# DTolm/VkFFT

Measured on NVIDIA H100. Metric: batched 1D C2C FP32 throughput (sample_0 sweep N=2^7..2^22, fwd+inv), higher is better.
Workload: dtype f32

## Files before the change

vkfft_b200/csrc/kernel_inst.cuh:

```cuda
#pragma once
#include <cstdio>

#include "kernel_registry.h"
#include "stockham.cuh"
#include "generic.cuh"
#include "pipe.cuh"
#include "fused4.cuh"
#include "ew.cuh"

#if !defined(B2_EMU)
#include <cuda_runtime.h>
#endif

namespace b200fft {

#if !defined(B2_EMU)
inline int launch_checked(const void* kernel, unsigned grid, unsigned threads, size_t smem, void* stream, const b2_pass_params* P) {
    void* args[] = {const_cast<b2_pass_params*>(P)};
    return (int)cudaLaunchKernel(kernel, dim3(grid), dim3(threads), args, smem, (cudaStream_t)stream);
}
#endif

template <int KIND> struct KindTraits;
template <> struct KindTraits<B2_KIND_ROWS> {
    static constexpr int LMAP = MAP_TFAST, SMAP = MAP_TFAST, LAYOUT = LAY_LINE;
    static constexpr bool IN_UNIT = true, OUT_UNIT = true;
};
template <> struct KindTraits<B2_KIND_ROWS_TOUT> {
    static constexpr int LMAP = MAP_TFAST, SMAP = MAP_QFAST, LAYOUT = LAY_LINE;
    static constexpr bool IN_UNIT = true, OUT_UNIT = false;
// ... 404 lines not shown
        for (int s = 0; s < SchB::ns; ++s) info.radices_b[s] = SchB::r(s);
        info.launch = &fused_launch_impl<CA, CB>;
        info.prepare = &fused_prepare_impl<CA, CB>;
        info.name = name;
        b2_register_fused(&info);
    }
};
template <bool EN, typename T, int TPLA, int QA, class SchA, int TPLB, int QB, class SchB, int REGS>
struct MaybeFused {
    explicit MaybeFused(const char*) {}
};
template <typename T, int TPLA, int QA, class SchA, int TPLB, int QB, class SchB, int REGS>
struct MaybeFused<true, T, TPLA, QA, SchA, TPLB, QB, SchB, REGS> {
    FusedRegistrar<T, false, TPLA, QA, SchA, TPLB, QB, SchB, REGS> f;
    FusedRegistrar<T, true, TPLA, QA, SchA, TPLB, QB, SchB, REGS> i;
    explicit MaybeFused(const char* n) : f(n), i(n) {}
};
}
#define B2_R(...) ::b200fft::RList<__VA_ARGS__>
#define B2_KF(shard, T, REGS, TPLA, QA, SA, TPLB, QB, SB)                                                  \
    static ::b200fft::MaybeFused<B2_SHARD_ON(shard), T, TPLA, QA, SA, TPLB, QB, SB, REGS>                  \
        B2_CAT(b2_regf_, __COUNTER__)("FUSED4<" #T ";A " #TPLA "x" #QA " " #SA ";B " #TPLB "x" #QB " " #SB ">");

namespace b200fft {
template <typename T, int Q, int REGS, bool INV, int N>
struct StagedRegistrar {
    using KT = KindTraits<B2_KIND_ROWS>;
    using C = KCfg<T, RList<N>, 1, Q, 1, KT::LMAP, KT::SMAP, KT::LAYOUT, INV, 0, KT::IN_UNIT, KT::OUT_UNIT, REGS, 10>;
    b2_kernel_info info;
    explicit StagedRegistrar(const char* name) {
        info = b2_kernel_info{};
        info.kind = B2_KIND_ROWS; info.prec = PrecOf<T>::value; info.n = N; info.inv = INV; info.ops = 0;
        info.threads = C::THREADS; info.q = Q; info.tpl = 1; info.v = 1; info.smem_bytes = C::SMEM_BYTES;
        info.ns = 1; info.radices[0] = N; info.lut_size = 0;
        info.launch = &launch_impl<C>;
        info.prepare = &prepare_impl<C>;
        info.name = name;
        b2_register_kernel(&info);
    }
};
template <bool EN, typename T, int Q, int REGS, int N>
struct MaybeStaged {
    explicit MaybeStaged(const char*) {}
};
template <typename T, int Q, int REGS, int N>
struct MaybeStaged<true, T, Q, REGS, N> {
// ... 25 lines not shown
```

vkfft_b200/csrc/kernel_registry.cpp:

```cpp
#include "kernel_registry.h"

#include <cstdio>
#include <cstdlib>
#include <cstring>
#include <vector>

namespace {
std::vector<b2_kernel_info*>& table() {
    static std::vector<b2_kernel_info*> t;
    return t;
}
int variant_override(int kind, int prec, int n) {
    const char* e = getenv("B200FFT_VARIANTS");
    if (!e) return 0;
    for (const char* p = e; *p;) {
        int k, pr, nn, v, used = 0;
        if (sscanf(p, "%d:%d:%d=%d%n", &k, &pr, &nn, &v, &used) == 4) {
            if (k == kind && pr == prec && nn == n) return v;
            p += used;
        } else {
            break;
        }
        if (*p == ',') ++p;
    }
// ... 42 lines not shown
}
extern "C" const b2_fused_info* b2_find_fused_variant(int prec, int n1, int n2, int inv, int variant) {
    for (const b2_fused_info* k : ftable())
        if (k->prec == prec && k->n1 == n1 && k->n2 == n2 && k->inv == inv && k->variant == variant) return k;
    return nullptr;
}
extern "C" const b2_fused_info* b2_find_fused(int prec, int n1, int n2, int inv) {
    int v = 0;
    if (const char* e = getenv("B200FFT_FUSED_VARIANTS")) {
        for (const char* p = e; *p;) {
            int a, b, vv, used = 0;
            if (sscanf(p, "%dx%d=%d%n", &a, &b, &vv, &used) == 3) {
                if (a == n1 && b == n2) v = vv;
                p += used;
            } else break;
            if (*p == ',') ++p;
        }
    }
    const b2_fused_info* k = v ? b2_find_fused_variant(prec, n1, n2, inv, v) : nullptr;
    return k ? k : b2_find_fused_variant(prec, n1, n2, inv, 0);
}
extern "C" int b2_fused_count(void) { return (int)ftable().size(); }
extern "C" const b2_fused_info* b2_fused_at(int i) { return ftable()[i]; }
```

vkfft_b200/csrc/kernel_registry.h:

```cpp
#pragma once
#include "pass_params.h"

#ifdef __cplusplus
extern "C" {
#endif

enum {
    B2_KIND_ROWS = 0,
    B2_KIND_ROWS_TOUT = 1,
    B2_KIND_COLS = 2,
    B2_KIND_GENERIC = 3,
    B2_KIND_ELEMENTWISE = 4,
    B2_KIND_COUNT
};
enum { B2_PREC_F32 = 0, B2_PREC_F64 = 1 };

typedef struct b2_kernel_info {
    int kind, prec, n, inv, ops;
    int variant;
    int pipelined;
    int threads, q, tpl, v, smem_bytes;
    int ns;
    int radices[8];
    int lut_size;
// ... 16 lines not shown
void b2_register_kernel(const b2_kernel_info* k);
const b2_kernel_info* b2_find_kernel(int kind, int prec, int n, int inv, int ops);
const b2_kernel_info* b2_find_kernel_variant(int kind, int prec, int n, int inv, int ops, int variant);
int b2_kernel_count(void);
const b2_kernel_info* b2_kernel_at(int i);

typedef struct b2_fused_info {
    int prec, n1, n2, inv;
    int variant;
    int threads, qa, qb, smem_bytes;
    int regs;
    int ns_a, ns_b;
    int radices_a[8], radices_b[8];
    int (*launch)(const b2_fused_params* F, unsigned max_ctas, void* stream);
    int (*prepare)(void);
    const char* name;
} b2_fused_info;
void b2_register_fused(const b2_fused_info* k);
const b2_fused_info* b2_find_fused(int prec, int n1, int n2, int inv);
const b2_fused_info* b2_find_fused_variant(int prec, int n1, int n2, int inv, int variant);
int b2_fused_count(void);
const b2_fused_info* b2_fused_at(int i);

#ifdef __cplusplus
}
#endif
```

vkfft_b200/csrc/kernels_shard.cu:

```cuda
#include "kernel_inst.cuh"

#ifndef B2_SHARD
#error "compile with -DB2_SHARD=<k>"
#endif

#include "kernel_list.def"
#include "kernel_list_nonpow2.def"
#include "kernel_list_blue1.def"
#include "kernel_list_fused.def"
```

vkfft_b200/csrc/pass_params.h:

```cpp
#pragma once
#include <stdint.h>

#ifdef __cplusplus
extern "C" {
#endif

enum {
    B2_MAX_OUTER = 3,
};

enum {
    B2_OP_NONE = 0,
    B2_OP_TWIDDLE_OUT = 1,
    B2_OP_SCALE = 2,
    B2_OP_MUL_IN = 4,
    B2_OP_MUL_OUT = 8,
    B2_OP_REAL_EVEN = 16,
    B2_OP_DCT23 = 32,
    B2_OP_PERM_IN = 64,
    B2_OP_BLUESTEIN = 256,
    B2_OP_CONV = 512,
    B2_OP_BLUE_FUSED = 1024,
    B2_OP_HALF_IN = 2048,
    B2_OP_HALF_OUT = 4096,
// ... 58 lines not shown
    uint32_t gen_flags;
} b2_pass_params;

enum {
    B2_GEN_FUSE_IN = 1,
    B2_GEN_FUSE_OUT = 2,
};

typedef struct b2_fused_params {
    unsigned long long tmap_a[16]
#if defined(__GNUC__) || defined(__CUDACC__)
        __attribute__((aligned(64)))
#endif
        ;
    b2_pass_params A, B;
    uint32_t* ctl;
    uint32_t nseq;
    uint32_t U, NU;
    uint32_t R;
    uint32_t TA, TB;
    uint32_t reserved;
} b2_fused_params;

enum {
    B2_FCTL_MAX_GROUPS = 1024,
    B2_FCTL_WORDS = 64 * B2_FCTL_MAX_GROUPS,
};

#ifdef __cplusplus
}
#endif
```

vkfft_b200/csrc/plan.h:

```cpp
#pragma once
#include <stdint.h>

#include <string>
#include <vector>

#include "../../include/b200fft.h"
#include "kernel_registry.h"
#include "pass_params.h"

namespace b200fft {

enum {
    R_SUCCESS = 0,
    R_MALLOC_FAILED = 1,
    R_PLAN_NOT_INITIALIZED = 4,
    R_NULL_TEMP_PASSED = 5,
    R_FFTDIM_GT_MAX = 7,
    R_INVALID_DEVICE = 1002,
    R_ONLY_FORWARD = 1006,
    R_ONLY_INVERSE = 1007,
    R_EMPTY_FFTDIM = 2001,
    R_EMPTY_SIZE = 2002,
    R_EMPTY_BUFFER = 2004,
    R_EMPTY_TEMPBUFFER = 2006,
// ... 27 lines not shown

struct AuxSpec {
    int prec, kind;
    uint64_t a, b;
};

struct PassPlan {
    const b2_kernel_info* k = nullptr;
    const b2_kernel_info* k_unaligned = nullptr;
    b2_pass_params P{};
    unsigned grid = 0;
    int in_role = ROLE_BUFFER, out_role = ROLE_BUFFER;
    int64_t in_off = 0, out_off = 0;
    int lut_id = -1;
    int lut_id_unaligned = -1;
    int tw_id = -1;
    int aux0_id = -1, aux1_id = -1;
    int aux0_role = -1;
    bool sync_before = false;
    bool in_scalar = false, out_scalar = false;
    const b2_fused_info* fused = nullptr;
    uint32_t fz_nseq = 0, fz_U = 0, fz_NU = 0, fz_R = 0, fz_TA = 0, fz_TB = 0, fz_L = 1;
    int lut_id_plain = -1;
    std::string note;
};

struct PlanGraph {
    b200fft_desc desc{};
    int prec = 0;
    uint64_t stride[B200FFT_MAX_DIMS] = {0, 0, 0, 0};
    uint64_t batches = 1;
    uint64_t batch_stride = 0;
    uint64_t total_elems = 0;
    uint64_t temp_elems = 0;
    bool has_fwd = false, has_inv = false;
    std::vector<PassPlan> fwd, inv;
    std::vector<LutSpec> luts;
    std::vector<TwSpec> tws;
    std::vector<AuxSpec> auxs;
    uint64_t temp_elems_real = 0;
    double flops = 0;
    uint64_t algorithmic_bytes = 0;
    uint32_t axis_uploads[2][B200FFT_MAX_DIMS] = {{0, 0, 0, 0}, {0, 0, 0, 0}};
    int skip_axis = -1;
    uint64_t ctl_words = 0;
    bool role_half[ROLE_COUNT] = {false, false, false, false, false};
// ... 7 lines not shown
```

vkfft_b200/csrc/planner.cpp:

```cpp
#include <algorithm>
#include <cmath>
#include <cstdio>
#include <cstdlib>
#include <cstring>

#include "lut.h"
#include "plan.h"

namespace b200fft {
namespace {

struct Dim {
    uint64_t n;
    int64_t is, os;
};

int lut_for(PlanGraph& g, const std::vector<int>& r) {
    for (size_t i = 0; i < g.luts.size(); ++i)
        if (g.luts[i].prec == g.prec && g.luts[i].radices == r) return (int)i;
    g.luts.push_back(LutSpec{g.prec, r});
    return (int)g.luts.size() - 1;
}
int tw_for(PlanGraph& g, uint64_t M) {
    for (size_t i = 0; i < g.tws.size(); ++i)
// ... 588 lines not shown
    if (a.P.nb[1] != 1 || a.P.nb[2] != 1 || (a.P.nb[0] > 1 && a.P.in_bs[0] != (int64_t)((uint64_t)a.P.n * b.P.n)) || a.P.in_gs != 1) return;
    const uint64_t N = (uint64_t)a.P.n * b.P.n, esz = esize(g), seq_bytes = N * esz;
    const uint64_t ga = (a.P.G + fk->qa - 1) / fk->qa, gb = (b.P.G + fk->qb - 1) / fk->qb;
    uint64_t K = std::max<uint64_t>(std::max(ga, gb) / 2, 8);
    if (seq_bytes >= (4ull << 20)) K = std::max(ga, gb);
    K = std::min<uint64_t>(K, 132);
    if (const char* e = getenv("B200FFT_FUSED_GROUP")) K = std::max<uint64_t>(1, strtoull(e, nullptr, 10));
    const uint64_t U = K, NU = 0, R = 2, L = 0;
    if (nseq * (ga + gb) > 0x7fffffffull) return;
    a.fused = fk;
    a.fz_nseq = (uint32_t)nseq; a.fz_U = (uint32_t)U; a.fz_NU = (uint32_t)NU; a.fz_R = (uint32_t)R;
    a.fz_TA = (uint32_t)ga; a.fz_TB = (uint32_t)gb; a.fz_L = (uint32_t)L;
    a.lut_id_plain = a.lut_id; b.lut_id_plain = b.lut_id;
    a.lut_id = lut_for(g, std::vector<int>(fk->radices_a, fk->radices_a + fk->ns_a));
    b.lut_id = lut_for(g, std::vector<int>(fk->radices_b, fk->radices_b + fk->ns_b));
    g.ctl_words = std::max<uint64_t>(g.ctl_words, B2_FCTL_WORDS);
    char buf[256];
    snprintf(buf, sizeof buf, " [fused with the next launch: %s, groups of %llu CTAs, %llu + %llu tiles per sequence]", fk->name,
             (unsigned long long)K, (unsigned long long)ga, (unsigned long long)gb);
    a.note += buf;
    b.note += " [runs inside the previous launch]";
}

int plan_c2c(PlanGraph& g, std::vector<PassPlan>& list, const C2CJob& job) {
    const uint64_t N = job.N;
    const int sc_ops = (job.scale != 1.0) ? B2_OP_SCALE : 0;
    std::vector<Dim> sliced = job.lines;
    int64_t slice_in = 0, slice_out = 0;
    if (job.line_world > 1) {
        bool done = false;
        for (size_t i = sliced.size(); i-- > 0 && !done;) {
            uint64_t first;
            if (sliced[i].n > 1 && sliced[i].n % job.line_world == 0) done = slice_dim(sliced[i], job.line_world, job.line_rank, slice_in, slice_out, first);
        }
        if (!done) return R_UNSUPPORTED_FFT_LENGTH;
    }
    std::vector<Dim> m = merge_dims(sliced);
    const bool contiguous = (job.es_in == 1 && job.es_out == 1);
    const int kind = job.unit_lines ? B2_KIND_COLS : B2_KIND_ROWS;
    const size_t first_launch = list.size();
    struct SyncMark {
        std::vector<PassPlan>& l; size_t at; bool on;
        ~SyncMark() { if (on && l.size() > at) l[at].sync_before = true; }
    } sync_mark{list, first_launch, job.sync_first};

    if (N == 1) return R_SUCCESS;
// ... 126 lines not shown
            a.tw_line0 = (uint32_t)first;
            a.sync_before = true;
            a.what = "distributed four-step 1/2 strided+phase (peer loads and stores)";
        }
        if ((rc = emit(g, list, a)) != R_SUCCESS) return rc;
        PassReq b;
        b.kind = B2_KIND_ROWS_TOUT; b.n = (int)N2; b.inv = job.inv; b.ops = sc_ops;
        b.in_es = 1; b.out_es = (int64_t)N1;
        b.group = Dim{N1, (int64_t)N2, 1};
        b.outer = s_tmp_out;
        b.in_role = ROLE_TEMP; b.out_role = job.out_role;
        b.in_base = job.tmp_base; b.out_base = job.out_base;
        b.scale = job.scale;
        b.what = "four-step 2/2 contiguous+transpose";
        if (dist) {
            uint64_t first;
            if (!slice_dim(b.group, job.world, job.rank, b.in_base, b.out_base, first)) return R_UNSUPPORTED_FFT_LENGTH;
            b.sync_before = true;
            b.what = "distributed four-step 2/2 contiguous+transpose (peer stores)";
        }
        const size_t ia = list.size() - 1;
        if ((rc = emit(g, list, b)) != R_SUCCESS) return rc;
        if (!dist && job.tmp_base % 16 == 0) try_fuse(g, list, ia);
        return R_SUCCESS;
    }
    const uint64_t N1 = f[0], N2 = f[1], N3 = f[2], M = N2 * N3;
    PassReq a;
    a.kind = B2_KIND_COLS; a.n = (int)N1; a.inv = job.inv; a.ops = B2_OP_TWIDDLE_OUT;
    a.in_es = (int64_t)M; a.out_es = (int64_t)M;
    a.group = Dim{M, 1, 1};
    const bool a_inplace = (job.in_role == ROLE_BUFFER) && !dist;
    a.outer = a_inplace ? s_in_in : s_in_tmp;
    a.in_role = job.in_role; a.out_role = a_inplace ? job.in_role : ROLE_TEMP;
    a.in_base = job.in_base; a.out_base = a_inplace ? job.in_base : job.tmp_base;
    a.twM = N;
    a.what = "four-step 1/3 strided+phase";
    if (dist) {
        uint64_t first;
        if (!slice_dim(a.group, job.world, job.rank, a.in_base, a.out_base, first)) return R_UNSUPPORTED_FFT_LENGTH;
        a.tw_line0 = (uint32_t)first;
        a.sync_before = true;
        a.what = "distributed four-step 1/3 strided+phase (peer loads and stores)";
    }
    if ((rc = emit(g, list, a)) != R_SUCCESS) return rc;
    PassReq b;
    b.kind = B2_KIND_COLS; b.n = (int)N2; b.inv = job.inv; b.ops = B2_OP_TWIDDLE_OUT;
// ... 749 lines not shown
```

vkfft_b200/csrc/runtime.cu:

```cuda
#include <cuda.h>
#include <cuda_runtime.h>

#include <cstdint>
#include <cstdio>
#include <cstdlib>
#include <cstring>
#include <new>
#include <string>
#include <vector>

#include "lut.h"
#include "plan.h"

using namespace b200fft;

struct TwDev {
    void* hi = nullptr;
    void* lo = nullptr;
    uint32_t shift = 0;
};

struct b200fft_plan {
    PlanGraph g;
    int device = 0;
// ... 123 lines not shown
    }
    p->d_auxs.assign(g.auxs.size(), nullptr);
    for (size_t i = 0; i < g.auxs.size() && rc == R_SUCCESS; ++i) {
        const AuxSpec& a = g.auxs[i];
        if (a.prec == B2_PREC_F32) rc = upload(make_aux<float>(a.kind, a.a, a.b), &p->d_auxs[i], p->lut_bytes);
        else rc = upload(make_aux<double>(a.kind, a.a, a.b), &p->d_auxs[i], p->lut_bytes);
    }
    if (rc == R_SUCCESS) {
        bool withdrawn = false;
        for (int dir = 0; dir < 2; ++dir)
            for (const PassPlan& pp : (dir ? g.inv : g.fwd))
                if (pp.k && pp.k->jit && b2_jit_prepare(pp.k) != 0) { b2_jit_disable(pp.k); withdrawn = true; }
        if (withdrawn) { cudaGetLastError(); free_plan(p); return b200fft_plan_create(desc, out); }
    }
    for (int dir = 0; dir < 2 && rc == R_SUCCESS; ++dir)
        for (const PassPlan& pp : (dir ? g.inv : g.fwd))
            if ((pp.k->prepare && pp.k->prepare() != 0) ||
                (pp.k_unaligned && pp.k_unaligned->prepare && pp.k_unaligned->prepare() != 0)) {
                rc = R_FAILED_TO_SET_DYNAMIC_SHARED_MEMORY;
                break;
            }
    for (int dir = 0; dir < 2 && rc == R_SUCCESS; ++dir)
        for (const PassPlan& pp : (dir ? g.inv : g.fwd))
            if (pp.fused && pp.fused->prepare && pp.fused->prepare() != 0) { rc = R_FAILED_TO_SET_DYNAMIC_SHARED_MEMORY; break; }
    if (rc == R_SUCCESS && g.ctl_words && cudaMalloc(&p->d_ctl, g.ctl_words * 4) != cudaSuccess) rc = R_FAILED_TO_ALLOCATE;
    if (rc == R_SUCCESS && g.temp_elems && !g.desc.user_temp_buffer) {
        p->temp_bytes = g.temp_elems * (g.role_half[ROLE_TEMP] ? 4 : (g.prec == B2_PREC_F64 ? 16 : 8));
        if (cudaMalloc(&p->d_temp, p->temp_bytes) != cudaSuccess) rc = R_FAILED_TO_ALLOCATE;
    }
    if (rc != R_SUCCESS) { cudaGetLastError(); free_plan(p); return rc; }
    *out = p;
    return R_SUCCESS;
}

static int exec_impl(b200fft_plan* p, int inverse, const b200fft_buffers* b, std::vector<cudaEvent_t>* marks, std::vector<int>* kinds);

extern "C" int b200fft_exec(b200fft_plan* p, int inverse, const b200fft_buffers* b) { return exec_impl(p, inverse, b, nullptr, nullptr); }

extern "C" int b200fft_debug_exec_timed(b200fft_plan* p, int inverse, const b200fft_buffers* b, float* ms, int* kind, int cap, int* count) {
    std::vector<cudaEvent_t> marks;
    std::vector<int> kinds;
    int rc = exec_impl(p, inverse, b, &marks, &kinds);
    if (rc == R_SUCCESS && cudaDeviceSynchronize() != cudaSuccess) rc = R_FAILED_TO_SYNCHRONIZE;
    int n = 0;
    for (size_t i = 0; i + 1 < marks.size() && rc == R_SUCCESS; ++i, ++n) {
        float t = 0;
        cudaEventElapsedTime(&t, marks[i], marks[i + 1]);
// ... 57 lines not shown
            P.tw_shift = p->d_tws[pp.tw_id].shift;
        }
    };
    const unsigned fused_max_ctas = [] { const char* e = getenv("B200FFT_FUSED_CTAS"); return e ? (unsigned)strtoul(e, nullptr, 10) : 0u; }();
    for (size_t ip = 0; ip < list.size(); ++ip) {
        const PassPlan& pp = list[ip];
        if (pp.fused && ip + 1 < list.size()) {
            mark(1);
            b2_fused_params F;
            memset(&F, 0, sizeof F);
            resolve(pp, F.A);
            resolve(list[ip + 1], F.B);
            if (const char* e = getenv("B200FFT_FUSED_FLAGS")) F.B.aux_u1 |= (uint32_t)strtoul(e, nullptr, 10);
            F.ctl = (uint32_t*)p->d_ctl;
            F.nseq = pp.fz_nseq; F.U = pp.fz_U; F.NU = pp.fz_NU; F.R = pp.fz_R; F.TA = pp.fz_TA; F.TB = pp.fz_TB; F.reserved = pp.fz_L;
            const bool aligned = ((((uintptr_t)F.A.in) | ((uintptr_t)F.B.in)) & 15) == 0;
            if (aligned && F.ctl && encode_pass_a_map(F, F.A.n, F.B.n, (uint32_t)pp.fused->qa)) {
                if (pp.fused->launch(&F, fused_max_ctas, (void*)st) != 0) return fail(R_FAILED_TO_LAUNCH_KERNEL);
                ++ip;
                continue;
            }
        }

        if (pp.sync_before) {
            mark(0);
            int brc = b200fft_window_barrier(p->window, (void*)st);
            if (brc != R_SUCCESS) return fail(brc);
        }
        mark(1);
        b2_pass_params P;
        resolve(pp, P);
        if (pp.lut_id_plain >= 0) P.lut = p->d_luts[pp.lut_id_plain];
        const b2_kernel_info* k = pp.k;
        if (k->pipelined && ((((uintptr_t)P.in) | (uintptr_t)(P.in_gs * (int64_t)esz) | (uintptr_t)(P.in_bs[0] * (int64_t)esz) |
                              (uintptr_t)(P.in_bs[1] * (int64_t)esz) | (uintptr_t)(P.in_bs[2] * (int64_t)esz)) & 15))
        {
            k = pp.k_unaligned;
            if (pp.lut_id_unaligned >= 0) P.lut = p->d_luts[pp.lut_id_unaligned];
        }
        if (!k || (k->jit ? b2_jit_launch(k, &P, pp.grid, (void*)st) : k->launch(&P, pp.grid, (void*)st)) != 0) {
            if (g.distributed) {
                for (size_t jp = ip + 1; jp < list.size(); ++jp)
                    if (list[jp].sync_before) b200fft_window_barrier(p->window, (void*)st);
                b200fft_window_barrier(p->window, (void*)st);
            }
            return fail(R_FAILED_TO_LAUNCH_KERNEL);
// ... 219 lines not shown
```

vkfft_b200/csrc/stockham.cuh:

```cuda
#pragma once
#include <math.h>

#include "pass_params.h"
#include "radix.cuh"

#if defined(B2_EMU)
#include "cuda_emu.h"
#else
#define B2_SMEM_LD(sm, i) ((sm)[(i)])
#define B2_SMEM_ST(sm, i, v) ((sm)[(i)] = (v))
#endif

namespace b200fft {

template <int... Rs>
struct RList {
    static constexpr int ns = sizeof...(Rs);
    B2_HD static constexpr int r(int s) {
        const int a[] = {Rs...};
        return a[s];
    }
    B2_HD static constexpr int S(int s) {
        int p = 1;
        for (int i = 0; i < s; ++i) p *= r(i);
        return p;
    }
    static constexpr int N = (Rs * ... * 1);
    B2_HD static constexpr int lut_off(int s) {
        int o = 0;
// ... 50 lines not shown
    static constexpr int TPL = TPL_;
    static constexpr int Q = Q_;
    static constexpr int V = V_;
    static constexpr int LMAP = LMAP_;
    static constexpr int SMAP = SMAP_;
    static constexpr int LAYOUT = LAYOUT_;
    static constexpr bool INV = INV_;
    static constexpr int OPS = OPS_;
    static constexpr bool IN_UNIT = IN_UNIT_;
    static constexpr bool OUT_UNIT = OUT_UNIT_;
    static constexpr int RMODE = RMODE_;
    static constexpr int THREADS = TPL * Q;
    static constexpr int MINB = (65536 / (THREADS * REGS_)) < 1 ? 1 : ((65536 / (THREADS * REGS_)) > 32 ? 32 : (65536 / (THREADS * REGS_)));
    static constexpr int PAD_SHIFT = (sizeof(T) == 4) ? 4 : 3;
    static constexpr int NPAD = N + (N >> PAD_SHIFT);
    static constexpr int LS = (LAYOUT == LAY_LINE) ? (Q == 1 ? NPAD : (NPAD | 1)) : 0;
    static constexpr int QP = Q;
    static constexpr int SMEM_ELEMS = RMODE == 10 ? Q * (N + 1)
                                    : ((Sch::ns <= 1 && RMODE != 1 && RMODE != 3 && RMODE != 4) ? 0 : ((LAYOUT == LAY_LINE) ? Q * LS : N * QP));
    static constexpr int SMEM_BYTES = SMEM_ELEMS * 2 * (int)sizeof(T);
    static constexpr bool TWCHAIN = true;
};

enum { XF_LDCG = 1, XF_DISCARD = 2 };

#if defined(__CUDA_ARCH__)
#define B2_OPAQUE64(v) asm("" : "+l"(v))
#else
#define B2_OPAQUE64(v) ((void)0)
#endif

#if defined(__CUDA_ARCH__)
template <typename T> B2_D cpx<T> ld_cg(const cpx<T>* p) {
    if constexpr (sizeof(T) == 4) { float2 v = __ldcg(reinterpret_cast<const float2*>(p)); return mk<T>(v.x, v.y); }
    else { double2 v = __ldcg(reinterpret_cast<const double2*>(p)); return mk<T>(v.x, v.y); }
}
#else
template <typename T> B2_D cpx<T> ld_cg(const cpx<T>* p) { return *p; }
#endif

struct NoHook { B2_D void operator()() const {} };

template <class C, int XF = 0, int ESI = 0, int ESO = 0>
struct Engine {
    using T = typename C::T;
    using X = cpx<T>;
    using Sch = typename C::Sch;
    static constexpr int N = C::N, TPL = C::TPL, Q = C::Q, V = C::V, NS = Sch::ns;
    static constexpr bool RUNNING_IN = !C::IN_UNIT && ESI == 0;
    static constexpr bool RUNNING_OUT = !C::OUT_UNIT && ESO == 0;
    static constexpr bool HIN = (C::ST & 1) != 0, HOUT = (C::ST & 2) != 0;
    static_assert(C::ST == 0 || (C::RMODE == 0 && V == 1 && sizeof(T) == 4 && XF == 0), "half storage: plain FP32 complex transforms");
    template <bool H, class A, class B> struct Sel { using type = A; };
    template <class A, class B> struct Sel<true, A, B> { using type = B; };
    using XI = typename Sel<HIN, X, uint32_t>::type;
    using XO = typename Sel<HOUT, X, uint32_t>::type;
    B2_D static X ldx(const X* p) { return *p; }
    B2_D static X ldx(const uint32_t* p) { float re, im; b2_h2_to_f2(*p, re, im); return mk<T>((T)re, (T)im); }
    B2_D static void stx(X* p, X a) { *p = a; }
    B2_D static void stx(uint32_t* p, X a) { *p = b2_f2_to_h2((float)a.x, (float)a.y); }

    B2_D static int sidx(int q, int p) {
        if constexpr (C::LAYOUT == LAY_LINE) return q * C::LS + p + (p >> C::PAD_SHIFT);
        else return p * C::QP + q;
// ... 367 lines not shown
            const X sum = a + bc, d = (a - bc) * ld_lut(w + k);
            X o = mk<T>(T(0.5) * (sum.x + d.y), T(0.5) * (sum.y - d.x));
            if (do_scale) o = o * sc;
            line[k] = o;
        }
    }

    template <int s>
    B2_D static void load_smem(X* x, const X* sm, int q, int t) {
        constexpr int r = Sch::r(s), NB = nbut<s>(), BPT = bpt<s>();
#pragma unroll
        for (int m = 0; m < BPT; ++m) {
#pragma unroll
            for (int v = 0; v < V; ++v) {
                const int b = V * (t + m * TPL) + v;
                if (guarded<s>() && b >= NB) continue;
#pragma unroll
                for (int k = 0; k < r; ++k) x[(m * V + v) * r + k] = B2_SMEM_LD(sm, sidx(q, b + k * NB));
            }
        }
    }

    template <int s>
    B2_D static void compute(X* x, const X* __restrict__ lut, int t) {
        constexpr int r = Sch::r(s), S = Sch::S(s), NB = nbut<s>(), BPT = bpt<s>();
#pragma unroll
        for (int m = 0; m < BPT; ++m) {
#pragma unroll
            for (int v = 0; v < V; ++v) {
                const int b = V * (t + m * TPL) + v;
                if (guarded<s>() && b >= NB) continue;
                X* xb = x + (m * V + v) * r;
                if constexpr (s > 0) {
                    const int j = b % S;
                    const X* l = lut + Sch::lut_off(s) + j;
                    if constexpr (B2_TW_CHAIN && C::TWCHAIN) {
                    X w[r];
#pragma unroll
                    for (int k = 1; k < r; ++k) {
                        if ((k & (k - 1)) == 0) w[k] = ld_lut(l + (k - 1) * S);
                        else w[k] = w[k & -k] * w[k - (k & -k)];
                        xb[k] = xb[k] * w[k];
                    }
                    } else {
#pragma unroll
                    for (int k = 1; k < r; ++k) xb[k] = xb[k] * ld_lut(l + (k - 1) * S);
// ... 1 lines not shown
                }
                dft<r, T>(xb);
            }
        }
    }

    template <int s>
    B2_D static void store_smem(const X* x, X* sm, int q, int t) {
        constexpr int r = Sch::r(s), S = Sch::S(s), NB = nbut<s>(), BPT = bpt<s>();
#pragma unroll
        for (int m = 0; m < BPT; ++m) {
#pragma unroll
            for (int v = 0; v < V; ++v) {
                const int b = V * (t + m * TPL) + v;
                if (guarded<s>() && b >= NB) continue;
                const int j = b % S;
                const int base = (b - j) * r + j;
#pragma unroll
                for (int k = 0; k < r; ++k) B2_SMEM_ST(sm, sidx(q, base + k * S), x[(m * V + v) * r + k]);
            }
        }
    }

    template <int s>
    B2_D static void store_global(const X* x, XO* __restrict__ line, int64_t es_rt, int t, bool valid,
                                  const b2_pass_params& P, uint32_t gline, uint32_t qline) {
        constexpr int r = Sch::r(s), NB = nbut<s>(), BPT = bpt<s>();
        static_assert(s == NS - 1, "global store only after the last stage");
        constexpr bool TW = (C::OPS & B2_OP_TWIDDLE_OUT) != 0;
        const bool do_scale = (P.ops & B2_OP_SCALE) != 0;
        const T sc = (T)P.scale;
        const int64_t es = C::OUT_UNIT ? 1 : (ESO ? (int64_t)ESO : es_rt);
        const int64_t step = (int64_t)NB * es;
        X s1 = mk<T>(T(1), T(0)), s2 = s1, s4 = s1;
        if constexpr (TW) {
            const uint64_t e1 = (uint64_t)gline * (uint64_t)NB;
            if constexpr (r > 1) s1 = twiddle2<T>((const X*)P.tw_hi, (const X*)P.tw_lo, P.tw_shift, e1);
            if constexpr (r > 2) s2 = twiddle2<T>((const X*)P.tw_hi, (const X*)P.tw_lo, P.tw_shift, 2 * e1);
            if constexpr (r > 4) s4 = twiddle2<T>((const X*)P.tw_hi, (const X*)P.tw_lo, P.tw_shift, 4 * e1);
        }
#pragma unroll
        for (int m = 0; m < BPT; ++m) {
            const int b0 = V * (t + m * TPL);
            const bool ok = valid && (!guarded<s>() || b0 < NB);
            if (!ok) continue;
            XO* dst = line + (int64_t)b0 * es;
            X w0[V], w2[V], w4[V], w6[V];
#pragma unroll
            for (int k = 0; k < r; ++k) {
// ... 1 lines not shown
                if constexpr (RUNNING_OUT) { if (k + 1 < r) { int64_t st = step; B2_OPAQUE64(st); dst += st; } }
                else sp = dst + k * step;
                X o[V];
#pragma unroll
                for (int v = 0; v < V; ++v) {
                    X a = x[(m * V + v) * r + k];
                    const int p = b0 + v + k * NB;
                    if constexpr (TW) {
                        const int tt = k & 7;
                        X w;
                        if (tt == 0) { w0[v] = twiddle2<T>((const X*)P.tw_hi, (const X*)P.tw_lo, P.tw_shift, (uint64_t)gline * (uint64_t)p); w = w0[v]; }
                        else if (tt == 1) w = w0[v] * s1;
                        else if (tt == 2) { w2[v] = w0[v] * s2; w = w2[v]; }
                        else if (tt == 3) w = w2[v] * s1;
                        else if (tt == 4) { w4[v] = w0[v] * s4; w = w4[v]; }
                        else if (tt == 5) w = w4[v] * s1;
                        else if (tt == 6) { w6[v] = w4[v] * s2; w = w6[v]; }
                        else w = w6[v] * s1;
                        a = a * w;
                    }
                    if (do_scale) a = a * sc;
                    o[v] = C::INV ? swp(a) : a;
                }
                if constexpr (V == 2 && C::OUT_UNIT && !HOUT) {
                    using G = typename gvec<T, 2>::type;
                    G g;
                    g.x = o[0].x; g.y = o[0].y; g.z = o[1].x; g.w = o[1].y;
                    *reinterpret_cast<G*>(sp) = g;
                } else {
#pragma unroll
                    for (int v = 0; v < V; ++v) stx(sp + (int64_t)v * es, o[v]);
                }
            }
        }
    }

    B2_D static void discard_tile(const b2_pass_params& P, int64_t obase_in, uint32_t grp, int tid) {
#if defined(__CUDA_ARCH__)
        static_assert(C::LAYOUT == LAY_LINE && C::IN_UNIT, "discard: contiguous input lines");
        constexpr int LINES_PER_ROW = (N * 2 * (int)sizeof(T)) / 128;
        static_assert(LINES_PER_ROW * 128 == N * 2 * (int)sizeof(T), "whole cache lines");
        const uint32_t g0 = grp * Q;
        const uint32_t nrows = (P.G - g0) < (uint32_t)Q ? (P.G - g0) : (uint32_t)Q;
        const char* base = (const char*)((const X*)P.in + obase_in + (int64_t)g0 * P.in_gs);
        if ((((uintptr_t)base) | (uintptr_t)(P.in_gs * 2 * (int64_t)sizeof(T))) & 127) return;
        for (uint32_t i = tid; i < nrows * LINES_PER_ROW; i += C::THREADS) {
            const char* a = base + (int64_t)(i / LINES_PER_ROW) * P.in_gs * 2 * (int64_t)sizeof(T) + (size_t)(i % LINES_PER_ROW) * 128;
// ... 295 lines not shown
```

Before: 8447.

## Fuse four-step column and row passes into one thread-block-cluster launch via DSMEM

Adds a Cluster4 kernel that runs both passes of a two-pass four-step FFT in one launch. Pass A writes its twiddled column outputs directly into the shared memory of peer CTAs in the cluster with mapa/st.shared::cluster, and pass B reads its rows from local shared memory. This removes the global-memory round trip of the intermediate buffer and one kernel launch. In exchange it adds cluster-wide barriers, scattered remote shared-memory stores and occupancy limits from cluster scheduling. It applies only to FP32 two-pass plans that have a matching registered cluster variant.

Result: faster. 8811, median of 6 (+4.3%).

```diff
diff --git a/vkfft_b200/csrc/cluster4.cuh b/vkfft_b200/csrc/cluster4.cuh
--- /dev/null
+++ b/vkfft_b200/csrc/cluster4.cuh
@@ -0,0 +1,146 @@
+#pragma once
+#include "stockham.cuh"
+
+namespace b200fft {
+
+#if defined(__CUDA_ARCH__)
+B2_D void cl_sync() {
+    asm volatile("barrier.cluster.arrive.release.aligned;\n\tbarrier.cluster.wait.acquire.aligned;" ::: "memory");
+}
+B2_D uint32_t cl_smem_addr(const void* p) { return (uint32_t)__cvta_generic_to_shared(p); }
+template <typename T>
+B2_D void cl_store(uint32_t local_addr, uint32_t rank, const cpx<T>& v) {
+    uint32_t a;
+    asm volatile("mapa.shared::cluster.u32 %0, %1, %2;" : "=r"(a) : "r"(local_addr), "r"(rank));
+    if constexpr (sizeof(T) == 4) asm volatile("st.shared::cluster.v2.f32 [%0], {%1, %2};" ::"r"(a), "f"(v.x), "f"(v.y) : "memory");
+    else asm volatile("st.shared::cluster.v2.f64 [%0], {%1, %2};" ::"r"(a), "d"(v.x), "d"(v.y) : "memory");
+}
+#elif defined(B2_EMU_CLUSTER)
+B2_D void cl_sync() { b2emu::cluster_sync(); }
+B2_D uint32_t cl_smem_addr(const void*) { return 0; }
+template <typename T>
+B2_D void cl_store(uint32_t local_addr, uint32_t rank, const cpx<T>& v) { b2emu::dsmem_st(rank, local_addr, v); }
+#elif defined(B2_EMU)
+#error "cluster kernels run on the emulation with thread-block clusters only (B2_EMU_CLUSTER, cuda_emu_cluster.h)"
+#else
+B2_D void cl_sync() {}
+B2_D uint32_t cl_smem_addr(const void*) { return 0; }
+template <typename T>
+B2_D void cl_store(uint32_t, uint32_t, const cpx<T>&) {}
+#endif
+
+template <class CA, class CB, int CL>
+struct Cluster4 {
+    using T = typename CA::T;
+    using X = cpx<T>;
+    using EA = Engine<CA, XF_DSMEM_OUT, CB::N, CB::N>;
+    using EB = Engine<CB, XF_SMEM_IN, 0, CA::N>;
+    static constexpr int N1 = CA::N, N2 = CB::N;
+    static constexpr int COLS = N2 / CL, ROWS = N1 / CL;
+    static constexpr int TA = COLS / CA::Q;
+    static constexpr int THREADS = TA * CA::THREADS;
+    static constexpr int TB = ROWS / CB::Q;
+    static constexpr int GB = THREADS / CB::THREADS;
+    static constexpr int TILE_A = CA::N * CA::Q;
+    static constexpr int ELEMS = (TA * TILE_A > ROWS * CB::LS) ? TA * TILE_A : ROWS * CB::LS;
+    static constexpr int SMEM_BYTES = ELEMS * (int)sizeof(X);
+    static_assert(CA::LAYOUT == LAY_ELEM && CB::LAYOUT == LAY_LINE, "pass A: interleaved columns, pass B: contiguous rows");
+    static_assert(CA::V == 1 && CB::V == 1 && (CA::OPS & B2_OP_TWIDDLE_OUT) != 0 && CA::INV == CB::INV, "plain Four-Step pair");
+    static_assert(N2 % CL == 0 && N1 % CL == 0 && COLS % CA::Q == 0 && ROWS % CB::Q == 0, "whole tiles per CTA");
+    static_assert(THREADS % CB::THREADS == 0 && TB % GB == 0 && THREADS <= 1024, "pass B runs in whole rounds of the CTA's threads");
+
+    B2_D static void seq_coords(const b2_pass_params& P, uint32_t seq, uint32_t& o0, uint32_t& o1, uint32_t& o2) {
+        o0 = seq % P.nb[0]; seq /= P.nb[0];
+        o1 = seq % P.nb[1]; seq /= P.nb[1];
+        o2 = seq;
+    }
+
+    struct RowSink {
+        uint32_t base;
+        uint32_t pcol;
+        B2_D void operator()(int p, const X& v) const {
+            const uint32_t idx = (uint32_t)(p % ROWS) * CB::LS + pcol;
+            cl_store<T>(base + idx * (uint32_t)sizeof(X), (uint32_t)(p / ROWS), v);
+        }
+    };
+
+    B2_D static void run(const b2_cluster_params& K, unsigned char* smem_raw) {
+        X* sm = reinterpret_cast<X*>(smem_raw);
+        const int tid = threadIdx.x;
+        const uint32_t rank = blockIdx.x % CL, seq = blockIdx.x / CL;
+        {
+            const b2_pass_params& P = K.A;
+            uint32_t o0, o1, o2;
+            seq_coords(P, seq, o0, o1, o2);
+            const int64_t obase = (int64_t)o0 * P.in_bs[0] + (int64_t)o1 * P.in_bs[1] + (int64_t)o2 * P.in_bs[2];
+            const X* __restrict__ lut = (const X*)P.lut;
+            const int g = tid / CA::THREADS, lt = tid % CA::THREADS;
+            X* sa = sm + (size_t)g * TILE_A;
+            const uint32_t col0 = rank * COLS + g * CA::Q;
+            using Sch = typename CA::Sch;
+            int ql, tl;
+            EA::template tmap<CA::LMAP>(lt, ql, tl);
+            {
+                X x[EA::template bpt<0>() * Sch::r(0)];
+                EA::template load_global<0>(x, (const X*)P.in + obase + (int64_t)(col0 + ql) * P.in_gs, P.in_es, tl, true);
+                EA::template compute<0>(x, lut, tl);
+                EA::template store_smem<0>(x, sa, ql, tl);
+            }
+            __syncthreads();
+            EA::template middle<1>(sa, lut, lt);
+            constexpr int s = Sch::ns - 1;
+            int qs, ts;
+            EA::template tmap<CA::SMAP>(lt, qs, ts);
+            X x[EA::template bpt<s>() * Sch::r(s)];
+            EA::template load_smem<s>(x, sa, qs, ts);
+            EA::template compute<s>(x, lut, ts);
+            cl_sync();
+            const uint32_t col = col0 + qs;
+            EA::template store_global<s>(x, nullptr, 0, ts, true, P, EA::twl(P, col, o0, o1, o2), (uint32_t)qs,
+                                         RowSink{cl_smem_addr(sm), col + (col >> CB::PAD_SHIFT)});
+        }
+        cl_sync();
+        {
+            const b2_pass_params& P = K.B;
+            uint32_t o0, o1, o2;
+            seq_coords(P, seq, o0, o1, o2);
+            const int64_t obase = (int64_t)o0 * P.out_bs[0] + (int64_t)o1 * P.out_bs[1] + (int64_t)o2 * P.out_bs[2];
+            const X* __restrict__ lut = (const X*)P.lut;
+            const int lt = tid % CB::THREADS;
+            using Sch = typename CB::Sch;
+            constexpr int s = Sch::ns - 1;
+            int ql, tl, qs, ts;
+            EB::template tmap<CB::LMAP>(lt, ql, tl);
+            EB::template tmap<CB::SMAP>(lt, qs, ts);
+#pragma unroll 1
+            for (int j = tid / CB::THREADS; j < TB; j += GB) {
+                X* sb = sm + (size_t)j * CB::Q * CB::LS;
+                {
+                    X x[EB::template bpt<0>() * Sch::r(0)];
+                    EB::template load_first_smem<0>(x, sb, ql, tl);
+                    EB::template compute<0>(x, lut, tl);
+                    __syncthreads();
+                    EB::template store_smem<0>(x, sb, ql, tl);
+                }
+                __syncthreads();
+                EB::template middle<1>(sb, lut, lt);
+                const uint32_t gs = rank * ROWS + j * CB::Q + qs;
+                X x[EB::template bpt<s>() * Sch::r(s)];
+                EB::template load_smem<s>(x, sb, qs, ts);
+                EB::template compute<s>(x, lut, ts);
+                EB::template store_global<s>(x, (X*)P.out + obase + (int64_t)gs * P.out_gs, P.out_es, ts, true, P,
+                                             EB::twl(P, gs, o0, o1, o2), (uint32_t)qs);
+            }
+        }
+    }
+};
+
+#if defined(__CUDACC__)
+template <class CA, class CB, int CL, int MINB>
+__global__ void __launch_bounds__(Cluster4<CA, CB, CL>::THREADS, MINB) cluster4_kernel(const __grid_constant__ b2_cluster_params K) {
+    extern __shared__ __align__(128) unsigned char b2_smem_cluster[];
+    Cluster4<CA, CB, CL>::run(K, b2_smem_cluster);
+}
+#endif
+
+}
diff --git a/vkfft_b200/csrc/kernel_inst.cuh b/vkfft_b200/csrc/kernel_inst.cuh
--- a/vkfft_b200/csrc/kernel_inst.cuh
+++ b/vkfft_b200/csrc/kernel_inst.cuh
@@ -6,6 +6,9 @@
 #include "generic.cuh"
 #include "pipe.cuh"
 #include "fused4.cuh"
+#if !defined(B2_EMU) || defined(B2_EMU_CLUSTER)
+#include "cluster4.cuh"
+#endif
 #include "ew.cuh"
 
 #if !defined(B2_EMU)
@@ -456,6 +459,105 @@
     static ::b200fft::MaybeFused<B2_SHARD_ON(shard), T, TPLA, QA, SA, TPLB, QB, SB, REGS>                  \
         B2_CAT(b2_regf_, __COUNTER__)("FUSED4<" #T ";A " #TPLA "x" #QA " " #SA ";B " #TPLB "x" #QB " " #SB ">");
 
+#if !defined(B2_EMU) || defined(B2_EMU_CLUSTER)
+namespace b200fft {
+#if defined(B2_EMU)
+template <class CA, class CB, int CL, int MINB>
+int cluster_launch_impl(const b2_cluster_params* K, void*) {
+    using CK = Cluster4<CA, CB, CL>;
+    const b2_cluster_params KK = *K;
+    b2emu::launch_cluster(KK.nseq * CL, CL, CK::THREADS, CK::SMEM_BYTES, [&](unsigned char* sm) { CK::run(KK, sm); }, b2emu::st().log);
+    return emu_refused();
+}
+template <class CA, class CB, int CL, int MINB> int cluster_prepare_impl() { return 0; }
+template <class CA, class CB, int CL, int MINB> int cluster_max_active_impl(int) { return b2emu::st().cluster_capable ? 1 : 0; }
+#else
+template <class CA, class CB, int CL, int MINB>
+cudaLaunchConfig_t cluster_config(unsigned grid, cudaLaunchAttribute* at, void* stream) {
+    cudaLaunchConfig_t cfg = {};
+    cfg.gridDim = dim3(grid);
+    cfg.blockDim = dim3(Cluster4<CA, CB, CL>::THREADS);
+    cfg.dynamicSmemBytes = Cluster4<CA, CB, CL>::SMEM_BYTES;
+    cfg.stream = (cudaStream_t)stream;
+    at[0].id = cudaLaunchAttributeClusterDimension;
+    at[0].val.clusterDim.x = CL; at[0].val.clusterDim.y = 1; at[0].val.clusterDim.z = 1;
+    cfg.attrs = at;
+    cfg.numAttrs = 1;
+    return cfg;
+}
+template <class CA, class CB, int CL, int MINB>
+int cluster_launch_impl(const b2_cluster_params* K, void* stream) {
+    cudaLaunchAttribute at[1];
+    const cudaLaunchConfig_t cfg = cluster_config<CA, CB, CL, MINB>(K->nseq * CL, at, stream);
+    return (int)cudaLaunchKernelEx(&cfg, cluster4_kernel<CA, CB, CL, MINB>, *K);
+}
+template <class CA, class CB, int CL, int MINB>
+int cluster_prepare_impl() {
+    int rc = (int)cudaFuncSetAttribute(cluster4_kernel<CA, CB, CL, MINB>, cudaFuncAttributeMaxDynamicSharedMemorySize,
+                                       Cluster4<CA, CB, CL>::SMEM_BYTES);
+    if (rc == 0 && CL > 8) rc = (int)cudaFuncSetAttribute(cluster4_kernel<CA, CB, CL, MINB>, cudaFuncAttributeNonPortableClusterSizeAllowed, 1);
+    return rc;
+}
+template <class CA, class CB, int CL, int MINB>
+int cluster_max_active_impl(int device) {
+    static int known[64] = {0};
+    if (device < 0 || device >= 64) return 0;
+    if (known[device]) return known[device] - 1;
+    int prev = -1;
+    if (cudaGetDevice(&prev) != cudaSuccess) { cudaGetLastError(); return 0; }
+    if (prev != device && cudaSetDevice(device) != cudaSuccess) { cudaGetLastError(); return 0; }
+    int n = 0;
+    cudaLaunchAttribute at[1];
+    const cudaLaunchConfig_t cfg = cluster_config<CA, CB, CL, MINB>(132 * CL, at, nullptr);
+    if (cluster_prepare_impl<CA, CB, CL, MINB>() != 0 ||
+        cudaOccupancyMaxActiveClusters(&n, (const void*)cluster4_kernel<CA, CB, CL, MINB>, &cfg) != cudaSuccess)
+        n = 0;
+    cudaGetLastError();
+    if (prev != device) cudaSetDevice(prev);
+    known[device] = 1 + (n > 0 ? n : 0);
+    return n > 0 ? n : 0;
+}
+#endif
+
+template <typename T, bool INV, int CL, int MINB, int TPLA, int QA, class SchA, int TPLB, int QB, class SchB>
+struct ClusterRegistrar {
+    using KA = KindTraits<B2_KIND_COLS>;
+    using KB = KindTraits<B2_KIND_ROWS_TOUT>;
+    using CA = KCfg<T, SchA, TPLA, QA, 1, KA::LMAP, KA::SMAP, KA::LAYOUT, INV, B2_OP_TWIDDLE_OUT, KA::IN_UNIT, KA::OUT_UNIT, 128, 0>;
+    using CB = KCfg<T, SchB, TPLB, QB, 1, KB::LMAP, KB::SMAP, KB::LAYOUT, INV, 0, KB::IN_UNIT, KB::OUT_UNIT, 128, 0>;
+    using CK = Cluster4<CA, CB, CL>;
+    b2_cluster_info info;
+    explicit ClusterRegistrar(const char* name) {
+        info = b2_cluster_info{};
+        info.prec = PrecOf<T>::value; info.n1 = SchA::N; info.n2 = SchB::N; info.inv = INV;
+        info.cluster = CL; info.threads = CK::THREADS; info.smem_bytes = CK::SMEM_BYTES;
+        info.tpl_a = TPLA; info.q_a = QA; info.tpl_b = TPLB; info.q_b = QB;
+        info.ns_a = SchA::ns; info.ns_b = SchB::ns;
+        for (int s = 0; s < SchA::ns; ++s) info.radices_a[s] = SchA::r(s);
+        for (int s = 0; s < SchB::ns; ++s) info.radices_b[s] = SchB::r(s);
+        info.launch = &cluster_launch_impl<CA, CB, CL, MINB>;
+        info.prepare = &cluster_prepare_impl<CA, CB, CL, MINB>;
+        info.max_active = &cluster_max_active_impl<CA, CB, CL, MINB>;
+        info.name = name;
+        b2_register_cluster(&info);
+    }
+};
+template <bool EN, typename T, int CL, int MINB, int TPLA, int QA, class SchA, int TPLB, int QB, class SchB>
+struct MaybeCluster {
+    explicit MaybeCluster(const char*) {}
+};
+template <typename T, int CL, int MINB, int TPLA, int QA, class SchA, int TPLB, int QB, class SchB>
+struct MaybeCluster<true, T, CL, MINB, TPLA, QA, SchA, TPLB, QB, SchB> {
+    ClusterRegistrar<T, false, CL, MINB, TPLA, QA, SchA, TPLB, QB, SchB> f;
+    ClusterRegistrar<T, true, CL, MINB, TPLA, QA, SchA, TPLB, QB, SchB> i;
+    explicit MaybeCluster(const char* n) : f(n), i(n) {}
+};
+}
+#define B2_KCL(shard, T, CL, MINB, TPLA, QA, SA, TPLB, QB, SB)                                               \
+    static ::b200fft::MaybeCluster<B2_SHARD_ON(shard), T, CL, MINB, TPLA, QA, SA, TPLB, QB, SB>              \
+        B2_CAT(b2_regcl_, __COUNTER__)("CLUSTER4<" #T ";" #CL " CTAs;A " #TPLA "x" #QA " " #SA ";B " #TPLB "x" #QB " " #SB ">");
+#endif
+
 namespace b200fft {
 template <typename T, int Q, int REGS, bool INV, int N>
 struct StagedRegistrar {
diff --git a/vkfft_b200/csrc/kernel_registry.cpp b/vkfft_b200/csrc/kernel_registry.cpp
--- a/vkfft_b200/csrc/kernel_registry.cpp
+++ b/vkfft_b200/csrc/kernel_registry.cpp
@@ -88,3 +88,40 @@
 }
 extern "C" int b2_fused_count(void) { return (int)ftable().size(); }
 extern "C" const b2_fused_info* b2_fused_at(int i) { return ftable()[i]; }
+
+namespace {
+std::vector<b2_cluster_info*>& ctable() {
+    static std::vector<b2_cluster_info*> t;
+    return t;
+}
+}
+extern "C" void b2_register_cluster(const b2_cluster_info* k) {
+    b2_cluster_info* m = const_cast<b2_cluster_info*>(k);
+    int v = 0;
+    for (const b2_cluster_info* o : ctable())
+        if (o->prec == k->prec && o->n1 == k->n1 && o->n2 == k->n2 && o->inv == k->inv) ++v;
+    m->variant = v;
+    ctable().push_back(m);
+}
+extern "C" const b2_cluster_info* b2_find_cluster(int prec, int n1, int n2, int inv) {
+    int v = 0;
+    if (const char* e = getenv("B200FFT_CLUSTER4_VARIANTS")) {
+        for (const char* p = e; *p;) {
+            int a, b, vv, used = 0;
+            if (sscanf(p, "%dx%d=%d%n", &a, &b, &vv, &used) == 3) {
+                if (a == n1 && b == n2) v = vv;
+                p += used;
+            } else break;
+            if (*p == ',') ++p;
+        }
+    }
+    const b2_cluster_info* dflt = nullptr;
+    for (const b2_cluster_info* k : ctable()) {
+        if (k->prec != prec || k->n1 != n1 || k->n2 != n2 || k->inv != inv) continue;
+        if (k->variant == v) return k;
+        if (k->variant == 0) dflt = k;
+    }
+    return dflt;
+}
+extern "C" int b2_cluster_count(void) { return (int)ctable().size(); }
+extern "C" const b2_cluster_info* b2_cluster_at(int i) { return ctable()[i]; }
diff --git a/vkfft_b200/csrc/kernel_registry.h b/vkfft_b200/csrc/kernel_registry.h
--- a/vkfft_b200/csrc/kernel_registry.h
+++ b/vkfft_b200/csrc/kernel_registry.h
@@ -62,6 +62,23 @@
 int b2_fused_count(void);
 const b2_fused_info* b2_fused_at(int i);
 
+typedef struct b2_cluster_info {
+    int prec, n1, n2, inv;
+    int variant;
+    int cluster, threads, smem_bytes;
+    int tpl_a, q_a, tpl_b, q_b;
+    int ns_a, ns_b;
+    int radices_a[8], radices_b[8];
+    int (*launch)(const b2_cluster_params* K, void* stream);
+    int (*prepare)(void);
+    int (*max_active)(int device);
+    const char* name;
+} b2_cluster_info;
+void b2_register_cluster(const b2_cluster_info* k);
+const b2_cluster_info* b2_find_cluster(int prec, int n1, int n2, int inv);
+int b2_cluster_count(void);
+const b2_cluster_info* b2_cluster_at(int i);
+
 #ifdef __cplusplus
 }
 #endif
diff --git a/vkfft_b200/csrc/kernels_shard.cu b/vkfft_b200/csrc/kernels_shard.cu
--- a/vkfft_b200/csrc/kernels_shard.cu
+++ b/vkfft_b200/csrc/kernels_shard.cu
@@ -8,3 +8,4 @@
 #include "kernel_list_nonpow2.def"
 #include "kernel_list_blue1.def"
 #include "kernel_list_fused.def"
+#include "kernel_list_cluster.def"
diff --git a/vkfft_b200/csrc/pass_params.h b/vkfft_b200/csrc/pass_params.h
--- a/vkfft_b200/csrc/pass_params.h
+++ b/vkfft_b200/csrc/pass_params.h
@@ -104,6 +104,11 @@
     uint32_t reserved;
 } b2_fused_params;
 
+typedef struct b2_cluster_params {
+    b2_pass_params A, B;
+    uint32_t nseq;
+} b2_cluster_params;
+
 enum {
     B2_FCTL_MAX_GROUPS = 1024,
     B2_FCTL_WORDS = 64 * B2_FCTL_MAX_GROUPS,
diff --git a/vkfft_b200/csrc/plan.h b/vkfft_b200/csrc/plan.h
--- a/vkfft_b200/csrc/plan.h
+++ b/vkfft_b200/csrc/plan.h
@@ -73,6 +73,8 @@
     const b2_fused_info* fused = nullptr;
     uint32_t fz_nseq = 0, fz_U = 0, fz_NU = 0, fz_R = 0, fz_TA = 0, fz_TB = 0, fz_L = 1;
     int lut_id_plain = -1;
+    const b2_cluster_info* cluster = nullptr;
+    uint32_t cl_nseq = 0;
     std::string note;
 };
 
diff --git a/vkfft_b200/csrc/planner.cpp b/vkfft_b200/csrc/planner.cpp
--- a/vkfft_b200/csrc/planner.cpp
+++ b/vkfft_b200/csrc/planner.cpp
@@ -634,6 +634,43 @@
     b.note += " [runs inside the previous launch]";
 }
 
+void try_cluster(PlanGraph& g, std::vector<PassPlan>& list, size_t ia) {
+    const char* off = getenv("B200FFT_NO_CLUSTER4");
+    if ((off && *off && *off != '0') || ia + 2 != list.size() || half_plan(g) || g.prec != B2_PREC_F32) return;
+    PassPlan& a = list[ia];
+    PassPlan& b = list[ia + 1];
+    if (a.fused || a.sync_before || b.sync_before || a.in_scalar || b.out_scalar) return;
+    if (!a.k || !b.k || a.k->jit || b.k->jit || a.k->pipelined || b.k->pipelined || a.k->kind != B2_KIND_COLS || b.k->kind != B2_KIND_ROWS_TOUT) return;
+    if (a.k->ops != B2_OP_TWIDDLE_OUT || b.k->ops != 0 || a.k->inv != b.k->inv || a.k->v != 1 || b.k->v != 1) return;
+    const b2_cluster_info* ck = b2_find_cluster(g.prec, (int)a.P.n, (int)b.P.n, a.k->inv);
+    if (!ck) return;
+    if (ck->tpl_a != a.k->tpl || ck->q_a != a.k->q || ck->tpl_b != b.k->tpl || ck->q_b != b.k->q || ck->ns_a != a.k->ns ||
+        ck->ns_b != b.k->ns)
+        return;
+    for (int s = 0; s < ck->ns_a; ++s) if (ck->radices_a[s] != a.k->radices[s]) return;
+    for (int s = 0; s < ck->ns_b; ++s) if (ck->radices_b[s] != b.k->radices[s]) return;
+    const int64_t n1 = a.P.n, n2 = b.P.n;
+    if (a.P.G != (uint32_t)n2 || b.P.G != (uint32_t)n1 || a.P.in_gs != 1 || a.P.in_es != n2 || b.P.out_gs != 1 || b.P.out_es != n1) return;
+    if (a.P.tw_sel != 0 || b.P.tw_sel != 0 || a.P.tw_line0 != 0) return;
+    uint64_t nseq = 1, nseq_b = 1;
+    for (int d = 0; d < B2_MAX_OUTER; ++d) { nseq *= a.P.nb[d]; nseq_b *= b.P.nb[d]; }
+    if (nseq != nseq_b || nseq * (uint64_t)ck->cluster > 0x7fffffffull) return;
+    if (a.in_role == b.out_role) {
+        if (a.in_off != b.out_off) return;
+        for (int d = 0; d < B2_MAX_OUTER; ++d)
+            if (a.P.nb[d] != b.P.nb[d] || (a.P.nb[d] > 1 && a.P.in_bs[d] != b.P.out_bs[d])) return;
+    }
+    if (ck->max_active(g.desc.device) <= 0) return;
+    a.cluster = ck;
+    a.cl_nseq = (uint32_t)nseq;
+    char buf[256];
+    snprintf(buf, sizeof buf, " [one cluster launch with the next pass: %s, clusters of %d CTAs]", ck->name, ck->cluster);
+    const size_t at = a.note.find(" n=");
+    if (at != std::string::npos) a.note = "four-step 1/2+2/2 in one cluster launch" + a.note.substr(at);
+    a.note += buf;
+    b.note += " [runs inside the previous launch]";
+}
+
 int plan_c2c(PlanGraph& g, std::vector<PassPlan>& list, const C2CJob& job) {
     const uint64_t N = job.N;
     const int sc_ops = (job.scale != 1.0) ? B2_OP_SCALE : 0;
@@ -806,6 +843,7 @@
         const size_t ia = list.size() - 1;
         if ((rc = emit(g, list, b)) != R_SUCCESS) return rc;
         if (!dist && job.tmp_base % 16 == 0) try_fuse(g, list, ia);
+        if (!dist) try_cluster(g, list, ia);
         return R_SUCCESS;
     }
     const uint64_t N1 = f[0], N2 = f[1], N3 = f[2], M = N2 * N3;
diff --git a/vkfft_b200/csrc/runtime.cu b/vkfft_b200/csrc/runtime.cu
--- a/vkfft_b200/csrc/runtime.cu
+++ b/vkfft_b200/csrc/runtime.cu
@@ -169,7 +169,10 @@
             }
     for (int dir = 0; dir < 2 && rc == R_SUCCESS; ++dir)
         for (const PassPlan& pp : (dir ? g.inv : g.fwd))
-            if (pp.fused && pp.fused->prepare && pp.fused->prepare() != 0) { rc = R_FAILED_TO_SET_DYNAMIC_SHARED_MEMORY; break; }
+            if ((pp.fused && pp.fused->prepare && pp.fused->prepare() != 0) || (pp.cluster && pp.cluster->prepare() != 0)) {
+                rc = R_FAILED_TO_SET_DYNAMIC_SHARED_MEMORY;
+                break;
+            }
     if (rc == R_SUCCESS && g.ctl_words && cudaMalloc(&p->d_ctl, g.ctl_words * 4) != cudaSuccess) rc = R_FAILED_TO_ALLOCATE;
     if (rc == R_SUCCESS && g.temp_elems && !g.desc.user_temp_buffer) {
         p->temp_bytes = g.temp_elems * (g.role_half[ROLE_TEMP] ? 4 : (g.prec == B2_PREC_F64 ? 16 : 8));
@@ -273,6 +276,18 @@
             }
         }
 
+        if (pp.cluster && ip + 1 < list.size()) {
+            mark(1);
+            b2_cluster_params K;
+            memset(&K, 0, sizeof K);
+            resolve(pp, K.A);
+            resolve(list[ip + 1], K.B);
+            K.nseq = pp.cl_nseq;
+            if (pp.cluster->launch(&K, (void*)st) != 0) return fail(R_FAILED_TO_LAUNCH_KERNEL);
+            ++ip;
+            continue;
+        }
+
         if (pp.sync_before) {
             mark(0);
             int brc = b200fft_window_barrier(p->window, (void*)st);
diff --git a/vkfft_b200/csrc/stockham.cuh b/vkfft_b200/csrc/stockham.cuh
--- a/vkfft_b200/csrc/stockham.cuh
+++ b/vkfft_b200/csrc/stockham.cuh
@@ -4,7 +4,9 @@
 #include "pass_params.h"
 #include "radix.cuh"
 
-#if defined(B2_EMU)
+#if defined(B2_EMU_CLUSTER)
+#include "cuda_emu_cluster.h"
+#elif defined(B2_EMU)
 #include "cuda_emu.h"
 #else
 #define B2_SMEM_LD(sm, i) ((sm)[(i)])
@@ -101,7 +103,7 @@
     static constexpr bool TWCHAIN = true;
 };
 
-enum { XF_LDCG = 1, XF_DISCARD = 2 };
+enum { XF_LDCG = 1, XF_DISCARD = 2, XF_SMEM_IN = 4, XF_DSMEM_OUT = 8 };
 
 #if defined(__CUDA_ARCH__)
 #define B2_OPAQUE64(v) asm("" : "+l"(v))
@@ -119,6 +121,7 @@
 #endif
 
 struct NoHook { B2_D void operator()() const {} };
+struct NoSink { template <class X> B2_D void operator()(int, const X&) const {} };
 
 template <class C, int XF = 0, int ESI = 0, int ESO = 0>
 struct Engine {
@@ -532,6 +535,16 @@
     }
 
     template <int s>
+    B2_D static void load_first_smem(X* x, const X* sm, int q, int t) {
+        static_assert((XF & XF_SMEM_IN) != 0 && s == 0 && V == 1, "first stage from shared memory");
+        load_smem<s>(x, sm, q, t);
+        if constexpr (C::INV) {
+#pragma unroll
+            for (int i = 0; i < bpt<s>() * Sch::r(s); ++i) x[i] = swp(x[i]);
+        }
+    }
+
+    template <int s>
     B2_D static void compute(X* x, const X* __restrict__ lut, int t) {
         constexpr int r = Sch::r(s), S = Sch::S(s), NB = nbut<s>(), BPT = bpt<s>();
 #pragma unroll
@@ -579,9 +592,9 @@
         }
     }
 
-    template <int s>
+    template <int s, class Sink = NoSink>
     B2_D static void store_global(const X* x, XO* __restrict__ line, int64_t es_rt, int t, bool valid,
-                                  const b2_pass_params& P, uint32_t gline, uint32_t qline) {
+                                  const b2_pass_params& P, uint32_t gline, uint32_t qline, const Sink& sink = Sink{}) {
         constexpr int r = Sch::r(s), NB = nbut<s>(), BPT = bpt<s>();
         static_assert(s == NS - 1, "global store only after the last stage");
         constexpr bool TW = (C::OPS & B2_OP_TWIDDLE_OUT) != 0;
@@ -629,7 +642,10 @@
                     if (do_scale) a = a * sc;
                     o[v] = C::INV ? swp(a) : a;
                 }
-                if constexpr (V == 2 && C::OUT_UNIT && !HOUT) {
+                if constexpr ((XF & XF_DSMEM_OUT) != 0) {
+                    static_assert(V == 1 && !HOUT, "one output per butterfly leg, FP32 / FP64 elements");
+                    sink(b0 + k * NB, o[0]);
+                } else if constexpr (V == 2 && C::OUT_UNIT && !HOUT) {
                     using G = typename gvec<T, 2>::type;
                     G g;
                     g.x = o[0].x; g.y = o[0].y; g.z = o[1].x; g.w = o[1].y;
```
